# ScuffleCloud/SVT-AV1-mirror

Hardware: AMD Instinct MI355X
Metric: open-loop ME 64x64 superblocks/sec + achieved HBM GB/s, 4K preset-8 (higher is better)
Workload: dtype u8

## Files before the change

### include/svtme.h

```cpp
#ifndef SVTME_H
#define SVTME_H

#include <stdbool.h>
#include <stdint.h>

#ifdef __cplusplus
extern "C" {
#endif

#define SVTME_PU_COUNT 85
#define SVTME_MAX_LISTS 2
#define SVTME_MAX_REFS 4
#define SVTME_MAX_PA_ME_CAND 23
#define SVTME_MAX_PA_ME_MV 7
#define SVTME_MAX_SAD_VALUE (128u * 128u * 255u)
#define SVTME_SUB_SAD_SEARCH 0
#define SVTME_FULL_SAD_SEARCH 1
#define SVTME_ME_MCTF 1
#define SVTME_ME_OPEN_LOOP 3
#define SVTME_PAD_FULL 72
#define SVTME_PAD_QUARTER 32
#define SVTME_PAD_SIXTEENTH 16

typedef int32_t svtme_status;
// ... 202 lines not shown
svtme_status svtme_ticket_wait_timed(svtme_ctx *ctx, uint64_t ticket, float *gpu_ms, float *copy_ms);
void *svtme_host_alloc(uint64_t bytes);
void svtme_host_free(void *p);
svtme_status svtme_host_register(void *p, uint64_t bytes);
svtme_status svtme_host_unregister(void *p);
svtme_status svtme_reserve(svtme_ctx *ctx, uint32_t width, uint32_t height, uint32_t max_refs, uint32_t tickets);
svtme_status svtme_reserve_pictures(svtme_ctx *ctx, uint32_t width, uint32_t height, uint32_t count);
svtme_status svtme_set_timing(svtme_ctx *ctx, int enable);
uint32_t svtme_timing_read(svtme_ctx *ctx, float stage_ms[5]);
#define SVTME_PATH_NO_FUSED_HME 1u
#define SVTME_PATH_NO_L1_FULL 2u
#define SVTME_PATH_NO_L0_FULL 4u
#define SVTME_PATH_NO_FP_WIDE 8u
#define SVTME_PATH_SPLIT_PASS 16u
#define SVTME_PATH_NO_A1_GATE 32u
svtme_status svtme_set_paths(svtme_ctx *ctx, uint32_t paths);
void *svtme_device_records(svtme_ctx *ctx, uint64_t *bytes);
void *svtme_stream(svtme_ctx *ctx);

#define SVTME_DG_MAX_PAIRS 8
#define SVTME_DG_MAX_SA 128

typedef struct svtme_dg_pair {
    uint64_t cur_picture_number;
    uint64_t ref_picture_number;
} svtme_dg_pair;

typedef struct svtme_dg_sb {
    uint32_t sad;
    int16_t mv_x, mv_y;
// ... 118 lines not shown
```

### svt-av1-mirror_amd/csrc/svtme_host.cpp

```cpp
#include <hip/hip_runtime.h>

#include <algorithm>
#include <cstdarg>
#include <cstdio>
#include <cstdlib>
#include <chrono>
#include <condition_variable>
#include <cstring>
#include <map>
#include <mutex>
#include <string>
#include <vector>

#include "svtme_device.h"

extern "C" hipError_t svtme_launch_build_full(const void *src, uint32_t src_stride, int w, int h, int ten_bit,
                                              DevPlane dst, int left, int top, int rows, hipStream_t s);
extern "C" hipError_t svtme_launch_copy_words(const void *src, void *dst, uint32_t nwords, hipStream_t s);
extern "C" hipError_t svtme_launch_pack(const svtme_ref_record *d_recs, const svtme_sb_result *d_sb, uint32_t n_sb,
                                        uint32_t R, const svtme_pack_layout *L, void *d_out, hipStream_t s);
extern "C" hipError_t svtme_launch_build_down(DevPlane prev, DevPlane dst, int left, int top, int rows,
                                              hipStream_t s);
extern "C" hipError_t svtme_launch_stages(const DevJob *d_jobs, const DevJob *h_jobs, uint32_t n, hipStream_t s,
                                          hipEvent_t *ev, uint32_t *mask);
// ... 164 lines not shown
        return fail(SVTME_ERR_INSUFFICIENT_RESOURCES, "hipStreamCreate: %s", hipGetErrorString(e));
    }
    c->lanes[0].s = c->stream;
    if ((e = svtme_prime_pyramid()) != hipSuccess || (e = svtme_prime_pack()) != hipSuccess ||
        (e = svtme_prime_stages()) != hipSuccess || (e = svtme_prime_dg()) != hipSuccess ||
        (e = svtme_prime_tfsp()) != hipSuccess) {
        (void)hipStreamDestroy(c->stream);
        delete c;
        return fail(SVTME_ERR_UNDEFINED, "svtme_ctx_create: loading the kernels: %s", hipGetErrorString(e));
    }
    static const struct {
        const char *var;
        uint32_t bit;
    } env_paths[] = {{"SVTME_NO_FUSED_HME", SVTME_PATH_NO_FUSED_HME}, {"SVTME_NO_L1_FULL", SVTME_PATH_NO_L1_FULL},
                     {"SVTME_NO_L0_FULL", SVTME_PATH_NO_L0_FULL},       {"SVTME_NO_FP_WIDE", SVTME_PATH_NO_FP_WIDE},
                     {"SVTME_SPLIT_PASS", SVTME_PATH_SPLIT_PASS},     {"SVTME_NO_A1_GATE", SVTME_PATH_NO_A1_GATE}};
    for (const auto &e : env_paths)
        if (const char *v = getenv(e.var))
            if (*v && strcmp(v, "0") != 0)
                c->paths |= e.bit;
    if (const char *v = getenv("SVTME_UPLOAD_ZERO_COPY"))
        c->zero_copy = !(*v && strcmp(v, "0") == 0);
    const svtme_status ps = prepare(c);
    if (ps) {
        svtme_ctx_destroy(c);
        return ps;
    }
    *out = c;
    return SVTME_OK;
}

extern "C" svtme_status svtme_set_paths(svtme_ctx *c, uint32_t paths) {
    if (!c || (paths & ~63u))
        return fail(SVTME_ERR_BAD_PARAMETER, "svtme_set_paths: null ctx or unknown path bits 0x%x", paths);
    std::lock_guard<std::mutex> lk(c->mu);
    c->paths = paths;
    return SVTME_OK;
}

extern "C" void svtme_ctx_destroy(svtme_ctx *c) {
    if (!c)
        return;
    (void)hipSetDevice(c->device);
    for (auto &L : c->lanes)
        if (L.s)
            (void)hipStreamSynchronize(L.s);
    if (c->ustream)
        (void)hipStreamSynchronize(c->ustream);
// ... 1572 lines not shown
```

### svt-av1-mirror_amd/csrc/svtme_stages.hip

```cpp
#include <hip/hip_ext.h>
#include <cstdlib>
#include <type_traits>

#include "svtme_me_common.h"

extern "C" bool svtme_hme_rt(const svtme_controls *c);

namespace svtme {


#define STAGE_A_BUF_DW 1024
#define STAGE_B_BUF_DW 640

template <int ND, typename P>
__device__ __forceinline__ void rows_qsad(P rp, int bstride_dw, const uint8_t *src, int src_stride,
                                          int k0, int k1, uint32_t acc[4]) {
    constexpr int CH = 64 / ND;
    for (int kc = k0; kc < k1; kc += CH) {
        const int ke         = min(k1, kc + CH);
        unsigned long long a = 0;
#pragma unroll 2
        for (int k = kc; k < ke; k++) {
            const P rd         = rp + k * bstride_dw;
            const uint32_t *sd = (const uint32_t *)(src + k * src_stride);
// ... 1541 lines not shown
            const uint32_t cnt = (uint32_t)__builtin_popcount(cm);
            if (cnt < SVTME_MAX_PA_ME_CAND)
                ca[cnt] = 0;
            o->total_me_candidate_index[pu] = (uint8_t)cnt;
#pragma unroll
            for (int s2 = 0; s2 < 8; s2++) {
                if (!((slots >> s2) & 1u))
                    continue;
                uint32_t *dst = ((cm >> s2) & 1u) ? &o->me_mv_array[pu][(s2 >> 2 ? max_l0 : 0) + (s2 & 3)] : &st.sink;
                *dst          = mvs[s2];
            }
        }
    }
}

__device__ __forceinline__ void finish_sb_out(StC &st, const DevJob &dj, uint32_t sb_local, uint32_t bw, uint32_t bh) {
    static_assert(offsetof(svtme_sb_result, me_8x8_cost_variance) ==
                          offsetof(svtme_sb_result, me_distortion) + 4 * SVTME_PU_COUNT &&
                      offsetof(svtme_sb_result, stationary_block_present) ==
                          offsetof(svtme_sb_result, me_8x8_cost_variance) + 24 &&
                      sizeof(svtme_sb_result) == offsetof(svtme_sb_result, stationary_block_present) + 8,
                  "svtme_sb_result tail: 6 distortion words, then the GM flag bytes and padding");
    constexpr int NIMG = (int)(offsetof(svtme_sb_result, me_8x8_cost_variance) / 4);
    constexpr int WDIST = NIMG, WGM = NIMG + 6;
    const svtme_job &job = dj.job;
    const int tid = threadIdx.x, wid = tid >> 6, lane = tid & 63;
    const bool mctf = SF(job, me_type) == SVTME_ME_MCTF;
    const bool en8 = SF(job, enable_me_8x8) != 0, en16 = SF(job, enable_me_16x16) != 0;
    uint32_t *img      = (uint32_t *)&st.keys[0][0];
    svtme_sb_result *o = (svtme_sb_result *)img;
    uint32_t *ow       = (uint32_t *)(dj.out_sb + sb_local);
    if (wid >= 2) {
        const int t     = tid - 128;
        const int head  = (int)((16u - ((uint32_t)(uintptr_t)ow & 15u)) & 15u) >> 2;
        const int n16   = (NIMG - head) >> 2;
        const int tail0 = head + 4 * n16;
        for (int i = t; i < n16; i += 128) {
            const uint32_t *v = img + head + 4 * i;
            *(uint4 *)(ow + head + 4 * i) = make_uint4(v[0], v[1], v[2], v[3]);
        }
        if (t >= 128 - 8) {
            const int j = t - (128 - 8);
            if (j < head)
                ow[j] = img[j];
            else if (j >= 4 && tail0 + (j - 4) < NIMG)
                ow[tail0 + (j - 4)] = img[tail0 + (j - 4)];
        }
    } else if (wid == 0) {
        uint32_t w6 = 0;
        if (!mctf) {
            const uint32_t d8v  = o->me_distortion[21 + lane];
            const uint32_t d16v = lane < 16 ? o->me_distortion[5 + lane] : 0;
            const uint32_t d32v = lane < 4 ? o->me_distortion[1 + lane] : 0;
            const uint32_t d8 = wave_sum_u32(d8v), d16 = wave_sum_u32(d16v), d32 = wave_sum_u32(d32v);
            const uint32_t d64  = o->me_distortion[0];
            const uint64_t mean = d8 / 64;
            const int64_t diff  = (int64_t)d8v - (int64_t)mean;
            const uint64_t sq1  = (uint64_t)(diff * diff);
            const uint64_t sq   = ((uint64_t)wave_sum_u32((uint32_t)(sq1 >> 24)) << 24) +
                                (uint64_t)wave_sum_u32((uint32_t)(sq1 & 0xFFFFFFu));
            const uint32_t pix  = bw * bh;
            const uint32_t dd = lane == 2 ? d64 : lane == 3 ? d32 : lane == 4 ? d16 : d8;
// ... 53 lines not shown
                if (my < -active_th)
                    atomicAdd(&cnt[li][ri][1][0], 1u);
                else if (my > active_th)
                    atomicAdd(&cnt[li][ri][1][1], 1u);
                const int stt = low ? 0 : 4;
                stat          = absi(mx) <= stt && absi(my) <= stt;
            }
            const uint64_t stationary = (uint64_t)__popcll(__ballot(stat)), tot = (uint64_t)n_blk;
            wave_lds_fence();
            const bool over = lane < 32 && cntf[lane] > (tot / 2);
            const bool any  = __ballot(over) != 0ull;
            flags = (stationary > ((tot * 5) / 100) ? 1u : 0u) | (any ? 1u << 8 : 0u);
        }
        if (lane < 2)
            ow[WGM + lane] = lane == 0 ? flags : 0u;
    }}

__device__ __forceinline__ void finish_sb(StC &st, const DevJob &dj, uint32_t sb_local, uint32_t bw, uint32_t bh) {
    finish_sb_cands(st, dj, sb_local, bw, bh);
    __syncthreads();
    HME_SUB(20);
    finish_sb_out(st, dj, sb_local, bw, bh);
}

__device__ __forceinline__ void write_records(const StC &st, const DevJob &dj, uint32_t sb_local, int t, int nt) {
    static_assert(sizeof(svtme_ref_record) == 176 * 4, "svtme_ref_record: 176 dwords");
    svtme_ref_record *out = dj.out_records + (size_t)sb_local * dj.R;
    const int R = (int)dj.R, nr0 = (int)SF(dj.job, num_refs[0]);
    for (int i = t; i < R * 44; i += nt) {
        const int k = i / 44, q = i - 44 * k;
        const int s = k < nr0 ? k : 4 + (k - nr0);
        uint4 v     = ((const uint4 *)st.rec[s])[q];
        if (q < 22 && !st.searched[s]) {
            if (4 * q + 0 < 85) v.x = U32MAX;
            if (4 * q + 1 < 85) v.y = U32MAX;
            if (4 * q + 2 < 85) v.z = U32MAX;
            if (4 * q + 3 < 85) v.w = U32MAX;
        }
        if (q == 42) {
            v.z = (uint32_t)st.hme_sad[s];
            v.w = (uint32_t)(st.hme_sad[s] >> 32);
        } else if (q == 43) {
            v.x = (uint32_t)(uint16_t)st.sc_x[s] | ((uint32_t)(uint16_t)st.sc_y[s] << 16);
            v.y = st.zz[s];
            v.z = (uint32_t)st.searched[s] | ((uint32_t)st.do_ref[s] << 8) | ((uint32_t)st.tf_exit << 16);
            v.w = 0;
        }
        ((uint4 *)(out + k))[q] = v;
    }
}

template <bool SUMS>
__device__ __forceinline__ void stage_c_tail(StC &st, const DevJob &dj, uint32_t sb_local, uint32_t bw, uint32_t bh, uint32_t vmask) {
    const svtme_job &job    = dj.job;
    const svtme_controls &c = job.ctrl;
    const int tid = threadIdx.x, lane = tid & 63;
    const bool w0 = (tid >> 6) == 0;
    const bool sbr = dj.out_sb != nullptr;
    uint32_t *img  = (uint32_t *)&st.keys[0][0];
    if (SF(job, me_type) != SVTME_ME_MCTF && SF(c, enable_hme_flag) && SF(c, enable_me_hme_ref_pruning) && w0) {
        const int s = lane;
        uint32_t sum8 = 0;
        if (SUMS) {
            if (s < 8)
                sum8 = st.sum8[s];
        } else {
            for (int k = 0; k < 8; k++) {
                if (!(slot_valid(vmask, k) && st.do_ref[k]))
                    continue;
                const uint32_t t = wave_sum_u32(st.rec[k][21 + lane]);
// ... 5 lines not shown
        if (s < 8) {
            v = st.hme_sad[s];
            if (slot_valid(vmask, s)) {
                v             = st.do_ref[s] ? (uint64_t)sum8 : (uint64_t)SVTME_MAX_SAD_VALUE * 64;
                st.hme_sad[s] = v;
            }
        }
        const uint16_t th = (uint16_t)SF(c, prune_ref_if_me_sad_dev_bigger_than_th);
        if (th != (uint16_t)~0) {
            const uint64_t best = wave_min_u64(v);
            if (s < 8 && (s & 3) >= 1 && (v - best) * 100 > (th * best))
                st.do_ref[s] = 0;
        }
    }
    if (SUMS && sbr && !w0)
        for (int i = tid - 64; i < (int)(sizeof(svtme_sb_result) + 15) / 16; i += 192)
            ((uint4 *)img)[i] = make_uint4(0, 0, 0, 0);
    __syncthreads();
    HME_SUB(17);
    if (SUMS && sbr) {
        if (tid < 128)
            finish_sb_cands(st, dj, sb_local, bw, bh);
        else
            write_records(st, dj, sb_local, tid - 128, 128);
        HME_SUB(18);
        __syncthreads();
        HME_SUB(20);
        finish_sb_out(st, dj, sb_local, bw, bh);
        HME_SUB(21);
        return;
    }
    write_records(st, dj, sb_local, tid, 256);
    HME_SUB(18);
    if (sbr) {
        for (int i = tid; i < (int)(sizeof(svtme_sb_result) + 15) / 16; i += 256)
            ((uint4 *)img)[i] = make_uint4(0, 0, 0, 0);
        __syncthreads();
        HME_SUB(19);
        finish_sb(st, dj, sb_local, bw, bh);
        HME_SUB(21);
    }
}

template <bool SUB_ME>
__global__ void __launch_bounds__(256) __attribute__((amdgpu_waves_per_eu(4, 8))) k_stage_c(const DevBatch B) {
    __shared__ StC st;
    uint32_t sb_local;
    const DevJob &dj        = batch_job(B, xcd_remap(blockIdx.x, gridDim.x), &sb_local);
    const svtme_job &job    = dj.job;
    const svtme_controls &c = job.ctrl;
    const int tid = threadIdx.x, lane = tid & 63, wid = tid >> 6;
    const bool w0           = wid == 0;
    const SbGeo G           = sb_geo(dj, sb_local);
    const uint32_t ox = G.ox, oy = G.oy, bw = G.bw, bh = G.bh;
// ... 650 lines not shown
    put(k8, 21 + lane);
    if ((lane & 3) == 0)
        put(k16, 5 + (lane >> 2));
    if ((lane & 15) == 0)
        put(k32, 1 + (lane >> 4));
    if (lane == 63)
        put(k64, 0);
    if (lane < 6) {
        const uint32_t t[6] = {(uint32_t)v.hme_sad, (uint32_t)(v.hme_sad >> 32),
                               (uint32_t)(uint16_t)v.sc_x | ((uint32_t)(uint16_t)v.sc_y << 16), v.zz,
                               (uint32_t)v.searched | ((uint32_t)v.do_ref << 8) | ((uint32_t)v.tf_exit << 16), 0u};
        o[170 + lane] = t[lane];
    }
}

template <bool SUB, bool K32, int TQ = (SUB ? FP_TQ : 2), bool WIDE = false, int WHOLE = 7>
__device__ __forceinline__ void fp_slot(const DevJob &dj, const SbGeo &G, int s, const uint32_t (&src)[SUB ? 4 : 8][2],
                                        int by, int bx, uint64_t hme_sad, uint32_t zz, uint32_t rdiv, int16_t sc_x,
                                        int16_t sc_y, uint8_t dref, uint8_t tf_exit, int part, uint32_t parts,
                                        unsigned long long *kp, CSlot *cs, svtme_ref_record *rec = nullptr) {
    const int lane = threadIdx.x & 63;
    const int l = s >> 2, r = s & 3;
    const uint32_t ox = G.ox, oy = G.oy;
    if (!dref || tf_exit) {
        const CSlot cv{hme_sad, zz, sc_x, sc_y, 0, 0, 0, 0, 0, 0, dref, 0, tf_exit};
        if (part == 0 && lane == 0)
            *cs = cv;
        if (rec)
            direct_record(rec, cv, 0, 0, 0, 0);
        return;
    }
    const DevPlane &P = dj.ref[l][r].lv[0];
    PuMin<K32> M;
    M.clear();
    const FpArea A = fp_area(dj, G, s, zz, rdiv, sc_x, sc_y, [&](const uint8_t *g) {
        const int sh = (int)((uintptr_t)g & 3);
        uint32_t p8, p64;
        if constexpr (K32) {
            p8  = fp_probe32<SUB>(M, g, P.stride >> 2, src, by, bx);
            p64 = wave_sum_u32(p8);
// ... 838 lines not shown
    if (search) {
        uint32_t bs;
        int x, y;
        key_result(half ? kt : kb, &bs, &x, &y);
        SD = bs;
        X  = i16((x + xo) * 2);
        Y  = i16((y + yo) * 2);
    }
    if ((lane & 47) == 0) {
        b->hx[s][q]   = X;
        b->hy[s][q]   = Y;
        b->hsad[s][q] = SD;
    }
}

__device__ __forceinline__ void stage_e_body(StC &st, const DevJob &dj, uint32_t sb_local,
                                             const SbGeo &G, uint32_t vmask, const CSlot *cin,
                                             unsigned long long *kb, bool reset) {
    const svtme_job &job = dj.job;
    const int tid = threadIdx.x, wid = tid >> 6, lane = tid & 63;
    const int R = (int)dj.R, nr0 = (int)SF(job, num_refs[0]);
    if (tid < 8) {
        const int s    = tid;
        const int k    = s < 4 ? s : nr0 + (s - 4);
        const bool has = s < 4 ? s < nr0 : k < R;
        CSlot v{};
        if (has)
            v = cin[k];
        st.hme_sad[s]  = has ? v.hme_sad : U32MAX;
        st.zz[s]       = has ? v.zz : U32MAX;
        st.sc_x[s]     = has ? v.sc_x : 0;
        st.sc_y[s]     = has ? v.sc_y : 0;
        st.searched[s] = has ? v.searched : 0;
        st.do_ref[s]   = has ? v.do_ref : 0;
        if (!(has && v.searched))
            st.sum8[s] = 0;
        if (s == (nr0 > 0 ? 0 : 4))
            st.tf_exit = has ? v.tf_exit : 0;
    }
    for (int kk = wid; kk < R; kk += 4) {
        const int s      = kk < nr0 ? kk : 4 + (kk - nr0);
        const CSlot &v   = cin[kk];
        const bool srch  = v.searched != 0;
        const uint32_t wm = srch ? magic_u32((uint32_t)max(1, (int)v.w)) : 0u;
        auto decode = [&](int pu, uint32_t &sad, uint32_t &mv) {
            sad = U32MAX, mv = 0;
            if (srch) {
                const size_t e                = (size_t)kk * SVTME_PU_COUNT + pu;
                const unsigned long long key = kb[e];
                if (reset)
                    kb[e] = ~0ull;
                const uint32_t o = (uint32_t)key;
                sad              = (uint32_t)(key >> 32);
                int16_t mx, my;
                if (v.probe && o == 0) {
// ... 9 lines not shown
            }
            st.rec[s][pu]                  = sad;
            st.rec[s][SVTME_PU_COUNT + pu] = mv;
        };
        uint32_t sad, mv;
        decode(21 + lane, sad, mv);
        if (srch) {
            const uint32_t t = wave_sum_u32(sad);
            if (lane == 0)
                st.sum8[s] = t;
        }
        if (lane < 21)
            decode(lane, sad, mv);
    }
    __syncthreads();
    stage_c_tail<true>(st, dj, sb_local, G.bw, G.bh, vmask);
}

__global__ void __launch_bounds__(256) __attribute__((amdgpu_waves_per_eu(4, 8))) k_stage_e(const DevBatch B) {
    __shared__ StC st;
    uint32_t sb_local;
    const DevJob &dj     = batch_job(B, xcd_remap(blockIdx.x, gridDim.x), &sb_local);
    const SbGeo G        = sb_geo(dj, sb_local);
    const uint32_t vmask = valid_mask(dj.job);
    stage_e_body(st, dj, sb_local, G, vmask, dj.cslot + (size_t)sb_local * dj.R,
                 dj.keys + (size_t)sb_local * dj.R * SVTME_PU_COUNT, dj.parts > 1);
}

struct HmeA {
    Dec d;
    unsigned long long key[SVTME_A_N];
// ... 126 lines not shown
struct HmeSh {
    DevJob dj;
    BState bs;
    CSlot cin[8];
    SlotCentre cen[8];
    uint8_t tf_exit;
    union U {
        HmeA a;
        StC st;
    } u;
};

#define HME_PRIO_HI() __builtin_amdgcn_s_setprio(2)
#define HME_PRIO_LO() __builtin_amdgcn_s_setprio(0)
#define HME_WAVES_PER_EU 8
template <bool FP, bool SUB_ME, bool K32, bool RT = false>
__global__ void __launch_bounds__(256) __attribute__((amdgpu_waves_per_eu(HME_WAVES_PER_EU, HME_WAVES_PER_EU))) k_hme(const DevBatch B) {
    __shared__ HmeSh sh;
    const int tid = threadIdx.x, lane = tid & 63, wid = UNI(tid >> 6);
    uint32_t sb_local;
    const DevJob &gj = batch_job(B, xcd_remap(blockIdx.x, gridDim.x), &sb_local);
    {
        static_assert(sizeof(DevJob) % 16 == 0 && sizeof(DevJob) / 16 <= 256, "DevJob: one uint4 per thread");
        if (tid < (int)(sizeof(DevJob) / 16))
            ((uint4 *)&sh.dj)[tid] = ((const uint4 *)&gj)[tid];
    }
    __syncthreads();
    const DevJob &dj        = sh.dj;
    const svtme_job &job    = dj.job;
    const svtme_controls &c = job.ctrl;
    const SbGeo G           = sb_geo(dj, sb_local);
    const uint32_t vmask    = valid_mask(job);
    Dec &d                  = sh.u.a.d;
    const int16_t sox = i16(((int16_t)G.ox) >> 2), soy = i16(((int16_t)G.oy) >> 2);
    const int kh  = (int)(G.bh >> 2) >> 1;
    const int kh1 = (int)(G.bh >> 2);
    const bool zz_on = c.me_early_exit_th || c.me_safe_limit_zz_th;
    HME_STAMP(0);

    if (wid == 0) {
// ... 86 lines not shown
        const bool act    = lane < 16 && slot_valid(vmask, s) && tl_or_l0(job, s >> 2) && ds;
        const bool nd     = act && ((lane & 1) ? !(eet && zs < (eet >> 2)) : !(eet && zs < eet));
        const unsigned long long m = __ballot(nd);
        if (lane == 0)
            sh.u.a.need = (uint32_t)m;
        HME_PRIO_LO();
    } else if (wid == 1) {
        if (lane < SVTME_A_N)
            sh.u.a.key[lane] = ~0ull;
        const bool gate = !RT && c.prehme_enable && c.prehme_l1_early_exit && job.num_lists == 2 &&
                          c.hme_search_method != SVTME_FULL_SAD_SEARCH && !(dj.paths & SVTME_PATH_NO_A1_GATE);
        a1_table<RT ? 1 : 0>(sh.u.a, dj, vmask, sox, soy, kh, 0, 0, 0, gate);
    } else {
        if (c.enable_hme_level2_flag) {
            const DevPlane &F = dj.cur.lv[0];
            const int row = (tid - 128) >> 2, part = tid & 3;
            const u32x4a4 v = ldg4((const uint32_t *)(F.base + (ptrdiff_t)(G.oy + 2 * row) * F.stride + G.ox + 16 * part));
            ((uint4 *)sh.u.a.src1[row])[part] = make_uint4(v.x, v.y, v.z, v.w);
        }
        if (c.enable_hme_level1_flag && tid < 160) {
            const DevPlane &Q = dj.cur.lv[1];
            const int row = (tid - 128) >> 1, half = tid & 1;
            const u32x4a4 v = ldg4((const uint32_t *)(Q.base + (ptrdiff_t)((G.oy >> 1) + 2 * row) * Q.stride +
                                                      (G.ox >> 1) + 16 * half));
            ((uint4 *)sh.u.a.src4[row])[half] = make_uint4(v.x, v.y, v.z, v.w);
        }
    }
    HME_WAVE(0);
    __syncthreads();
    HME_STAMP(1);
    HME_STAMP(2);
    auto a1_tiles = [&]() {
        uint32_t sr[8][4];
        {
            const uint8_t *sp = uni_ptr(dj.cur.lv[2].base + (ptrdiff_t)soy * dj.cur.lv[2].stride + sox);
            const int sst     = UNI(dj.cur.lv[2].stride);
#pragma unroll
            for (int k = 0; k < 8; k++) {
                const uint4 v = sld4(sp + (ptrdiff_t)(2 * k) * sst);
                sr[k][0] = v.x, sr[k][1] = v.y, sr[k][2] = v.z, sr[k][3] = v.w;
            }
        }
        const int nitems = sh.u.a.nitems, nsrch = sh.u.a.nsrch;
        const uint32_t need = sh.u.a.need;
        const int pstride = dj.cur.lv[2].stride;
        const int nitems3 = sh.u.a.nitems3, base2 = sh.u.a.base2, end1 = sh.u.a.end1, base3 = sh.u.a.base3;
        auto tiles = [&](auto fullk, int lo, int hi, bool gated) {
            for (int it = lo + tid; it < hi; it += 256) {
                if (it >= nitems3 && it < base2)
                    continue;
                const HSrch &e = sh.u.a.srch[find_search(sh.u.a.srch, nsrch, it)];
                if (!((need >> e.need) & 1u))
                    continue;
                if (gated && a1_mirrored(sh.u.a, c, need, e.id))
                    continue;
                const int local = it - e.item0;
                const int rt = mdiv(local, e.ncm), col = local - rt * e.ncols;
                auto run = [&](auto TT) {
                    constexpr int T = decltype(TT)::value;
                    int yf, tv;
                    if (e.skip) {
                        yf = 2 * T * rt + 1;
                        tv = min(T, e.cnt0 - T * rt);
// ... 236 lines not shown
            e.item0     = incl - items;
            sh.u.a.s1[kpos] = e;
        }
        if (lane == 63)
            sh.u.a.nitems1 = incl;
        if (lane == 0)
            sh.u.a.nsrch1 = tot;
    }
    __syncthreads();
    HME_PRIO_LO();
    HME_STAMP(4);
    {
        const int nlanes = 4 * sh.u.a.nitems1, nsrch = sh.u.a.nsrch1;
        const int pstride = dj.cur.lv[1].stride;
        auto tiles = [&](auto fullk) {
            for (int it4 = tid; it4 < nlanes; it4 += 256) {
                const int it    = it4 >> 2;
                const HSrch1 &e = sh.u.a.s1[find_search(sh.u.a.s1, nsrch, it)];
                const int local = it - e.item0;
                const int y = mdiv(local, e.ncm), col = local - y * e.ncols;
                const unsigned long long kk = hme_tile32q<decltype(fullk)::value>(e.a0, pstride, HQ1 * col, e.sh,
                                                                                  e.sa_w, y, kh1, sh.u.a.src4);
                if ((it4 & 3) == 0 && kk != ~0ull)
                    atomicMin(&sh.u.a.key1[e.id], kk);
            }
        };
        tiles(std::false_type());
    }
    __syncthreads();
    if (wid == 0 && lane < 32 && sh.u.a.hsad[lane] == ~0ull) {
        uint32_t best;
// ... 40 lines not shown
            const int incl = wave_incl_scan(items);
            if (mk) {
                e.item0            = incl - items;
                sh.u.a.s1[kpos] = e;
            }
            if (lane == 63)
                sh.u.a.nitems1 = incl;
            if (lane == 0)
                sh.u.a.nsrch1 = tot;
        }
        __syncthreads();
        {
            const int nlanes = 8 * sh.u.a.nitems1, nsrch = sh.u.a.nsrch1;
            const int pstride = dj.cur.lv[0].stride;
            const int kh2     = (int)(G.bh >> 1);
            for (int it8 = tid; it8 < nlanes; it8 += 256) {
                const int it    = it8 >> 3;
                const HSrch1 &e = sh.u.a.s1[find_search(sh.u.a.s1, nsrch, it)];
                const int local = it - e.item0;
                const int y = mdiv(local, e.ncm), col = local - y * e.ncols;
                const unsigned long long kk = hme_tile64(e.a0, pstride, HQ * col, e.sh, e.sa_w, y, kh2, sh.u.a.src1);
                if ((it8 & 7) == 0 && kk != ~0ull)
                    atomicMin(&sh.u.a.key1[e.id], kk);
            }
        }
        __syncthreads();
        if (wid == 0 && lane < 32 && sh.u.a.hsad[lane] == ~0ull) {
            uint32_t best;
            int x, y;
            key_result(sh.u.a.key1[lane], &best, &x, &y);
            sh.u.a.hsad[lane] = hsub ? (uint64_t)best * 2 : best;
// ... 21 lines not shown
        HME_STAMP(6);
        return;
    }
    if (wid == 0) {
        HME_PRIO_HI();
        wave_lds_fence();
        const SlotCentre scv = final_centre(gj.job, &sh.bs, vmask);
        if (lane < 8)
            sh.cen[lane] = scv;
        if (lane == 0)
            sh.tf_exit = job.me_type == SVTME_ME_MCTF && scv.hme_sad < job.tf_me_exit_th;
    }
    __syncthreads();
    HME_PRIO_LO();
    HME_STOP(55);
    for (int k = wid; k < (int)dj.R; k += 4) {
        constexpr int ROWS = SUB_ME ? 4 : 8, RSTEP = SUB_ME ? 2 : 1;
        int fl = lane;
        asm volatile("" : "+v"(fl));
        const int z16 = fl >> 2, k4 = fl & 3;
        const int by  = ((z16 >> 3) << 2) | (((z16 >> 1) & 1) << 1) | (k4 >> 1);
        const int bx  = (((z16 >> 2) & 1) << 2) | ((z16 & 1) << 1) | (k4 & 1);
        const DevPlane &C = gj.cur.lv[0];
        const int cst     = UNI(C.stride);
        const __amdgpu_buffer_rsrc_t crs = plane_rsrc(uni_ptr(C.base + (ptrdiff_t)G.oy * cst + G.ox));
        const uint32_t coff = (uint32_t)(by * 8 * cst + bx * 8);
        uint32_t src[ROWS][2];
#pragma unroll
        for (int rr = 0; rr < ROWS; rr++) {
            const auto v = __builtin_amdgcn_raw_buffer_load_b64(crs, (int)coff, rr * RSTEP * cst, 0);
            src[rr][0] = v[0];
            src[rr][1] = v[1];
        }
        const int nr0       = (int)SF(gj.job, num_refs[0]);
        const int s         = k < nr0 ? k : 4 + (k - nr0);
        const SlotCentre &v = sh.cen[s];
        fp_slot<SUB_ME, K32, 2, false, HME_WHOLE>(gj, G, s, src, by, bx, rl64(v.hme_sad, 0), (uint32_t)UNI(v.zz), (uint32_t)UNI(v.reduce_div),
                                (int16_t)UNI(v.sc_x), (int16_t)UNI(v.sc_y), (uint8_t)UNI(v.do_ref),
                                (uint8_t)UNI(sh.tf_exit), 0, 1u, &sh.u.st.keys[k][0], &sh.cin[k]);
    }
    HME_WAVE(1);
    __syncthreads();
    HME_STAMP(6);
    stage_e_body(sh.u.st, gj, sb_local, G, vmask, sh.cin, &sh.u.st.keys[0][0], false);
    HME_STAMP(7);
}

}

extern "C" void svtme_stage_a_list(const svtme_job *job, uint8_t *list, uint32_t *count) {
    const svtme_controls &c = job->ctrl;
    uint32_t n = 0;
    for (int s = 0; s < 8; s++) {
        const int l = s >> 2, r = s & 3;
        if (l >= job->num_lists || r >= job->num_refs[l])
            continue;
        if (!(job->temporal_layer_index > 0 || l == 0))
            continue;
        const bool zz = c.me_early_exit_th || c.me_safe_limit_zz_th;
// ... 72 lines not shown
        for (int k = 0; k < 2; k++) {
            const uint32_t mw = (uint32_t)c.prehme_sa_cfg[k].sa_min.width * f, xw = c.prehme_sa_cfg[k].sa_max.width;
            const uint32_t mh = (uint32_t)c.prehme_sa_cfg[k].sa_min.height * f, xh = c.prehme_sa_cfg[k].sa_max.height;
            dj->ph_sa[s][k][0] = (int16_t)(uint16_t)(mw < xw ? mw : xw);
            dj->ph_sa[s][k][1] = (int16_t)(uint16_t)(mh < xh ? mh : xh);
        }
    }
}

extern "C" bool svtme_hme_fused(const svtme_job *job) {
    const svtme_controls &c = job->ctrl;
    return (job->width % 64) == 0 && c.hme_search_method != SVTME_FULL_SAD_SEARCH;
}
static bool hme_fused(const DevJob &dj) { return svtme_hme_fused(&dj.job) && !(dj.paths & SVTME_PATH_NO_FUSED_HME); }

extern "C" bool svtme_hme_rt(const svtme_controls *c) {
    return c->enable_me_sr_adjustment && c->distance_based_hme_resizing && c->reduce_hme_l0_sr_th_min &&
           c->reduce_hme_l0_sr_th_max;
}

extern "C" bool svtme_l1_full(const svtme_controls *c) {
    return c->hme_search_method == SVTME_FULL_SAD_SEARCH && c->enable_hme_flag && c->enable_hme_level1_flag &&
           !c->enable_hme_level2_flag && c->hme_l1_sa.width <= 16 && c->hme_l1_sa.height <= 16;
}
static bool l1_full(const DevJob &dj) { return svtme_l1_full(&dj.job.ctrl) && !(dj.paths & SVTME_PATH_NO_L1_FULL); }

extern "C" bool svtme_l0_full(const DevJob *dj) {
    const svtme_controls &c = dj->job.ctrl;
    if (c.hme_search_method != SVTME_FULL_SAD_SEARCH || c.prehme_enable || !c.enable_hme_flag ||
        !c.enable_hme_level0_flag || svtme_hme_rt(&c) || (dj->job.width % 64) % 16 != 0 ||
// ... 53 lines not shown
    if (fp_wide_lds(c, paths)) {
        parts = parts > (h + 7) / 8 ? parts : (h + 7) / 8;
        parts = (parts + 3) & ~3u;
    }
    return parts < 1 ? 1 : (parts > 16 ? 16 : parts);
}
extern "C" uint32_t svtme_fp_parts(const svtme_controls *c) { return svtme_fp_parts_paths(c, 0); }

extern "C" uint32_t svtme_launch_key(const DevJob *dj) {
    const bool full = dj->job.ctrl.me_search_method == SVTME_FULL_SAD_SEARCH;
    return (uint32_t)full | (uint32_t)(dj->parts != 0) << 1 | (uint32_t)svtme_fp_k32(&dj->job.ctrl) << 2 |
           (uint32_t)(dj->job.ctrl.enable_hme_level2_flag != 0) << 3 | (uint32_t)hme_fused(*dj) << 4 |
           (uint32_t)(dj->parts == 1) << 5 | (uint32_t)svtme_fp_wide(&dj->job.ctrl) << 6 |
           (uint32_t)svtme_hme_rt(&dj->job.ctrl) << 7 | (uint32_t)fp_wide_lds(*dj) << 8 |
           (uint32_t)l1_full(*dj) << 9 | (uint32_t)svtme_l0_full(dj) << 10 |
           (uint32_t)((dj->paths & SVTME_PATH_SPLIT_PASS) != 0) << 11;
}

static DevBatch make_batch(const DevJob *d_jobs, const DevJob *h, uint32_t n, uint32_t (*units)(const DevJob &)) {
    DevBatch b;
    b.jobs     = d_jobs;
    b.n        = n;
    uint32_t t = 0;
    for (uint32_t k = 0; k < SVTME_MAX_BATCH; k++) {
        b.start[k] = k < n ? t : 0xFFFFFFFFu;
        if (k < n)
            t += units(h[k]);
    }
    b.total = t;
    return b;
}

#define SVTME_LAUNCH(K, grid, k, ...)                                                                               \
    do {                                                                                                           \
        if (ev) {                                                                                                  \
            hipExtLaunchKernelGGL(K, grid, dim3(256), 0, s, ev[2 * (k)], ev[2 * (k) + 1], 0, __VA_ARGS__);           \
            *mask |= 1u << (k);                                                                                    \
        } else                                                                                                     \
            hipLaunchKernelGGL(K, grid, dim3(256), 0, s, __VA_ARGS__);                                             \
    } while (0)

extern "C" hipError_t svtme_prime_stages(void) {
    const void *k[] = {
        (const void *)svtme::k_hme<true, true, true, false>,   (const void *)svtme::k_hme<true, true, true, true>,
        (const void *)svtme::k_hme<false, true, true, false>,  (const void *)svtme::k_hme<true, true, false, false>,
        (const void *)svtme::k_stage_a<false>,                 (const void *)svtme::k_stage_a<true>,
        (const void *)svtme::k_stage_d<false>,                 (const void *)svtme::k_stage_d<true>,
        (const void *)svtme::k_stage_b<false>,                 (const void *)svtme::k_stage_b<true>,
        (const void *)svtme::k_stage_c<false>,                 (const void *)svtme::k_stage_c<true>,
        (const void *)svtme::k_stage_c1<true, true, true>,     (const void *)svtme::k_stage_c1<true, true>,
        (const void *)svtme::k_stage_c1<true, false>,          (const void *)svtme::k_stage_c1<false, true, true>,
        (const void *)svtme::k_stage_c1<false, true>,          (const void *)svtme::k_stage_c1<false, false>,
        (const void *)svtme::k_l0_full<2>,                     (const void *)svtme::k_l0_full<4>,
        (const void *)svtme::k_l1_full,                        (const void *)svtme::k_fp_wide,
        (const void *)svtme::k_stage_e};
    hipFuncAttributes a;
    for (const void *f : k) {
        const hipError_t e = hipFuncGetAttributes(&a, f);
        if (e != hipSuccess)
            return e;
// ... 8 lines not shown
    const DevJob &h0 = h_jobs[0];
    if (mask)
        *mask = 0;
    const DevBatch bd = make_batch(d_jobs, h_jobs, n, [](const DevJob &j) { return j.job.sb_count; });
    const bool full = h0.job.ctrl.me_search_method == SVTME_FULL_SAD_SEARCH;
    const bool k32  = svtme_fp_k32(&h0.job.ctrl);
    const bool rt = svtme_hme_rt(&h0.job.ctrl);
#define SVTME_HME(FP, SUB, K32)                                                                                     \
    do {                                                                                                           \
        if (rt)                                                                                                    \
            SVTME_LAUNCH((svtme::k_hme<FP, SUB, K32, true>), dim3(bd.total), 0, bd);                               \
        else                                                                                                       \
            SVTME_LAUNCH((svtme::k_hme<FP, SUB, K32, false>), dim3(bd.total), 0, bd);                              \
    } while (0)
    if (hme_fused(h0) && h0.parts == 1 && !(h0.paths & SVTME_PATH_SPLIT_PASS)) {
        if (full && k32)
            SVTME_HME(true, false, true);
        else if (full)
            SVTME_HME(true, false, false);
        else if (k32)
            SVTME_HME(true, true, true);
        else
            SVTME_HME(true, true, false);
        return hipGetLastError();
    }
    if (hme_fused(h0)) {
        SVTME_HME(false, true, true);
    } else {
    const DevBatch ba = make_batch(d_jobs, h_jobs, n, [](const DevJob &j) { return j.job.sb_count * j.ta_count; });
    bool short_l0 = true;
    for (uint32_t k = 0; k < n; k++)
// ... 63 lines not shown
```

### svt-av1-mirror_amd/svtme.py

```python
from __future__ import annotations

import ctypes as C
import os
from dataclasses import dataclass, field

import numpy as np

PKG_DIR = os.path.dirname(os.path.abspath(__file__))
REPO_DIR = os.path.dirname(PKG_DIR)

PU_COUNT = 85
MAX_SAD_VALUE = 128 * 128 * 255
MAX_TICKETS = 64
PAD_FULL, PAD_QUARTER, PAD_SIXTEENTH = 72, 32, 16
SUB_SAD_SEARCH, FULL_SAD_SEARCH = 0, 1
ME_MCTF, ME_OPEN_LOOP = 1, 3
PATH_NO_FUSED_HME, PATH_NO_L1_FULL, PATH_NO_L0_FULL, PATH_NO_FP_WIDE, PATH_SPLIT_PASS = 1, 2, 4, 8, 16
RES_240P, RES_360P, RES_480P, RES_720P, RES_1080P, RES_4K, RES_8K = range(7)


class Area(C.Structure):
    _fields_ = [("width", C.c_uint16), ("height", C.c_uint16)]


class AreaMinMax(C.Structure):
    _fields_ = [("sa_min", Area), ("sa_max", Area)]


class Controls(C.Structure):
    _fields_ = [
        ("hme_search_method", C.c_uint8),
        ("me_search_method", C.c_uint8),
# ... 893 lines not shown
```

Before: 68.62 million.

## Launch fused HME kernel with three wavefronts for sub-SAD low-ref jobs

Adds a 3-wavefront (192-thread) variant of the fused HME kernel, used by default for sub-SAD, non-RT jobs with at most four references. Work loops, the image store, record writes and the source loads are made generic over the wave count. Full-pel slot assignment now hands searched references round-robin to waves and gives unsearched slots to the last wave, so idle waves are not spent on them. The aim is more resident workgroups per CU with less idle-wave waste, at the cost of fewer threads per block for the per-SB tail work and a new HME_4WAVES opt-out flag.

```diff
diff --git a/include/svtme.h b/include/svtme.h
--- a/include/svtme.h
+++ b/include/svtme.h
@@ -240,6 +240,7 @@
 #define SVTME_PATH_NO_FP_WIDE 8u
 #define SVTME_PATH_SPLIT_PASS 16u
 #define SVTME_PATH_NO_A1_GATE 32u
+#define SVTME_PATH_HME_4WAVES 64u
 svtme_status svtme_set_paths(svtme_ctx *ctx, uint32_t paths);
 void *svtme_device_records(svtme_ctx *ctx, uint64_t *bytes);
 void *svtme_stream(svtme_ctx *ctx);
diff --git a/svt-av1-mirror_amd/csrc/svtme_host.cpp b/svt-av1-mirror_amd/csrc/svtme_host.cpp
--- a/svt-av1-mirror_amd/csrc/svtme_host.cpp
+++ b/svt-av1-mirror_amd/csrc/svtme_host.cpp
@@ -202,7 +202,8 @@
         uint32_t bit;
     } env_paths[] = {{"SVTME_NO_FUSED_HME", SVTME_PATH_NO_FUSED_HME}, {"SVTME_NO_L1_FULL", SVTME_PATH_NO_L1_FULL},
                      {"SVTME_NO_L0_FULL", SVTME_PATH_NO_L0_FULL},       {"SVTME_NO_FP_WIDE", SVTME_PATH_NO_FP_WIDE},
-                     {"SVTME_SPLIT_PASS", SVTME_PATH_SPLIT_PASS},     {"SVTME_NO_A1_GATE", SVTME_PATH_NO_A1_GATE}};
+                     {"SVTME_SPLIT_PASS", SVTME_PATH_SPLIT_PASS},     {"SVTME_NO_A1_GATE", SVTME_PATH_NO_A1_GATE},
+                     {"SVTME_HME_4WAVES", SVTME_PATH_HME_4WAVES}};
     for (const auto &e : env_paths)
         if (const char *v = getenv(e.var))
             if (*v && strcmp(v, "0") != 0)
@@ -219,7 +220,7 @@
 }
 
 extern "C" svtme_status svtme_set_paths(svtme_ctx *c, uint32_t paths) {
-    if (!c || (paths & ~63u))
+    if (!c || (paths & ~127u))
         return fail(SVTME_ERR_BAD_PARAMETER, "svtme_set_paths: null ctx or unknown path bits 0x%x", paths);
     std::lock_guard<std::mutex> lk(c->mu);
     c->paths = paths;
diff --git a/svt-av1-mirror_amd/csrc/svtme_stages.hip b/svt-av1-mirror_amd/csrc/svtme_stages.hip
--- a/svt-av1-mirror_amd/csrc/svtme_stages.hip
+++ b/svt-av1-mirror_amd/csrc/svtme_stages.hip
@@ -1579,6 +1579,7 @@
     }
 }
 
+template <int NW = 4>
 __device__ __forceinline__ void finish_sb_out(StC &st, const DevJob &dj, uint32_t sb_local, uint32_t bw, uint32_t bh) {
     static_assert(offsetof(svtme_sb_result, me_8x8_cost_variance) ==
                           offsetof(svtme_sb_result, me_distortion) + 4 * SVTME_PU_COUNT &&
@@ -1595,8 +1596,7 @@
     uint32_t *img      = (uint32_t *)&st.keys[0][0];
     svtme_sb_result *o = (svtme_sb_result *)img;
     uint32_t *ow       = (uint32_t *)(dj.out_sb + sb_local);
-    if (wid >= 2) {
-        const int t     = tid - 128;
+    auto store_image = [&](int t) {
         const int head  = (int)((16u - ((uint32_t)(uintptr_t)ow & 15u)) & 15u) >> 2;
         const int n16   = (NIMG - head) >> 2;
         const int tail0 = head + 4 * n16;
@@ -1611,6 +1611,9 @@
             else if (j >= 4 && tail0 + (j - 4) < NIMG)
                 ow[tail0 + (j - 4)] = img[tail0 + (j - 4)];
         }
+    };
+    if (wid >= 2) {
+        store_image(tid - 128);
     } else if (wid == 0) {
         uint32_t w6 = 0;
         if (!mctf) {
@@ -1694,13 +1697,17 @@
         }
         if (lane < 2)
             ow[WGM + lane] = lane == 0 ? flags : 0u;
-    }}
-
+        if (NW == 3)
+            store_image(64 + lane);
+    }
+}
+
+template <int NW = 4>
 __device__ __forceinline__ void finish_sb(StC &st, const DevJob &dj, uint32_t sb_local, uint32_t bw, uint32_t bh) {
     finish_sb_cands(st, dj, sb_local, bw, bh);
     __syncthreads();
     HME_SUB(20);
-    finish_sb_out(st, dj, sb_local, bw, bh);
+    finish_sb_out<NW>(st, dj, sb_local, bw, bh);
 }
 
 __device__ __forceinline__ void write_records(const StC &st, const DevJob &dj, uint32_t sb_local, int t, int nt) {
@@ -1730,10 +1737,11 @@
     }
 }
 
-template <bool SUMS>
+template <bool SUMS, int NW = 4>
 __device__ __forceinline__ void stage_c_tail(StC &st, const DevJob &dj, uint32_t sb_local, uint32_t bw, uint32_t bh, uint32_t vmask) {
     const svtme_job &job    = dj.job;
     const svtme_controls &c = job.ctrl;
+    constexpr int NT = 64 * NW;
     const int tid = threadIdx.x, lane = tid & 63;
     const bool w0 = (tid >> 6) == 0;
     const bool sbr = dj.out_sb != nullptr;
@@ -1769,7 +1777,7 @@
         }
     }
     if (SUMS && sbr && !w0)
-        for (int i = tid - 64; i < (int)(sizeof(svtme_sb_result) + 15) / 16; i += 192)
+        for (int i = tid - 64; i < (int)(sizeof(svtme_sb_result) + 15) / 16; i += NT - 64)
             ((uint4 *)img)[i] = make_uint4(0, 0, 0, 0);
     __syncthreads();
     HME_SUB(17);
@@ -1777,22 +1785,22 @@
         if (tid < 128)
             finish_sb_cands(st, dj, sb_local, bw, bh);
         else
-            write_records(st, dj, sb_local, tid - 128, 128);
+            write_records(st, dj, sb_local, tid - 128, NT - 128);
         HME_SUB(18);
         __syncthreads();
         HME_SUB(20);
-        finish_sb_out(st, dj, sb_local, bw, bh);
+        finish_sb_out<NW>(st, dj, sb_local, bw, bh);
         HME_SUB(21);
         return;
     }
-    write_records(st, dj, sb_local, tid, 256);
+    write_records(st, dj, sb_local, tid, NT);
     HME_SUB(18);
     if (sbr) {
-        for (int i = tid; i < (int)(sizeof(svtme_sb_result) + 15) / 16; i += 256)
+        for (int i = tid; i < (int)(sizeof(svtme_sb_result) + 15) / 16; i += NT)
             ((uint4 *)img)[i] = make_uint4(0, 0, 0, 0);
         __syncthreads();
         HME_SUB(19);
-        finish_sb(st, dj, sb_local, bw, bh);
+        finish_sb<NW>(st, dj, sb_local, bw, bh);
         HME_SUB(21);
     }
 }
@@ -2473,6 +2481,11 @@
     }
 }
 
+__device__ __forceinline__ CSlot fp_unsearched(uint64_t hme_sad, uint32_t zz, int16_t sc_x, int16_t sc_y, uint8_t dref,
+                                               uint8_t tf_exit) {
+    return CSlot{hme_sad, zz, sc_x, sc_y, 0, 0, 0, 0, 0, 0, dref, 0, tf_exit};
+}
+
 template <bool SUB, bool K32, int TQ = (SUB ? FP_TQ : 2), bool WIDE = false, int WHOLE = 7>
 __device__ __forceinline__ void fp_slot(const DevJob &dj, const SbGeo &G, int s, const uint32_t (&src)[SUB ? 4 : 8][2],
                                         int by, int bx, uint64_t hme_sad, uint32_t zz, uint32_t rdiv, int16_t sc_x,
@@ -2482,7 +2495,7 @@
     const int l = s >> 2, r = s & 3;
     const uint32_t ox = G.ox, oy = G.oy;
     if (!dref || tf_exit) {
-        const CSlot cv{hme_sad, zz, sc_x, sc_y, 0, 0, 0, 0, 0, 0, dref, 0, tf_exit};
+        const CSlot cv = fp_unsearched(hme_sad, zz, sc_x, sc_y, dref, tf_exit);
         if (part == 0 && lane == 0)
             *cs = cv;
         if (rec)
@@ -3351,6 +3364,7 @@
     }
 }
 
+template <int NW = 4>
 __device__ __forceinline__ void stage_e_body(StC &st, const DevJob &dj, uint32_t sb_local,
                                              const SbGeo &G, uint32_t vmask, const CSlot *cin,
                                              unsigned long long *kb, bool reset) {
@@ -3375,7 +3389,7 @@
         if (s == (nr0 > 0 ? 0 : 4))
             st.tf_exit = has ? v.tf_exit : 0;
     }
-    for (int kk = wid; kk < R; kk += 4) {
+    for (int kk = wid; kk < R; kk += NW) {
         const int s      = kk < nr0 ? kk : 4 + (kk - nr0);
         const CSlot &v   = cin[kk];
         const bool srch  = v.searched != 0;
@@ -3415,7 +3429,7 @@
             decode(lane, sad, mv);
     }
     __syncthreads();
-    stage_c_tail<true>(st, dj, sb_local, G.bw, G.bh, vmask);
+    stage_c_tail<true, NW>(st, dj, sb_local, G.bw, G.bh, vmask);
 }
 
 __global__ void __launch_bounds__(256) __attribute__((amdgpu_waves_per_eu(4, 8))) k_stage_e(const DevBatch B) {
@@ -3572,16 +3586,21 @@
 #define HME_PRIO_HI() __builtin_amdgcn_s_setprio(2)
 #define HME_PRIO_LO() __builtin_amdgcn_s_setprio(0)
 #define HME_WAVES_PER_EU 8
-template <bool FP, bool SUB_ME, bool K32, bool RT = false>
-__global__ void __launch_bounds__(256) __attribute__((amdgpu_waves_per_eu(HME_WAVES_PER_EU, HME_WAVES_PER_EU))) k_hme(const DevBatch B) {
+template <bool FP, bool SUB_ME, bool K32, bool RT = false, int NW = 4>
+__global__ void __launch_bounds__(64 * NW) __attribute__((amdgpu_waves_per_eu(HME_WAVES_PER_EU, HME_WAVES_PER_EU))) k_hme(const DevBatch B) {
+    static_assert(NW == 3 || NW == 4, "k_hme: 3 or 4 wavefronts");
+    static_assert(sizeof(HmeSh) <= 16384, "HmeSh: ten workgroups per CU (160 KB of LDS)");
+    constexpr int NT = 64 * NW;
     __shared__ HmeSh sh;
     const int tid = threadIdx.x, lane = tid & 63, wid = UNI(tid >> 6);
     uint32_t sb_local;
     const DevJob &gj = batch_job(B, xcd_remap(blockIdx.x, gridDim.x), &sb_local);
     {
-        static_assert(sizeof(DevJob) % 16 == 0 && sizeof(DevJob) / 16 <= 256, "DevJob: one uint4 per thread");
+        static_assert(sizeof(DevJob) % 16 == 0 && sizeof(DevJob) / 16 <= 2 * NT, "DevJob: at most two uint4 per thread");
         if (tid < (int)(sizeof(DevJob) / 16))
             ((uint4 *)&sh.dj)[tid] = ((const uint4 *)&gj)[tid];
+        if (sizeof(DevJob) / 16 > NT && tid + NT < (int)(sizeof(DevJob) / 16))
+            ((uint4 *)&sh.dj)[tid + NT] = ((const uint4 *)&gj)[tid + NT];
     }
     __syncthreads();
     const DevJob &dj        = sh.dj;
@@ -3698,9 +3717,18 @@
     } else {
         if (c.enable_hme_level2_flag) {
             const DevPlane &F = dj.cur.lv[0];
-            const int row = (tid - 128) >> 2, part = tid & 3;
-            const u32x4a4 v = ldg4((const uint32_t *)(F.base + (ptrdiff_t)(G.oy + 2 * row) * F.stride + G.ox + 16 * part));
-            ((uint4 *)sh.u.a.src1[row])[part] = make_uint4(v.x, v.y, v.z, v.w);
+            constexpr int NP = 128 / (NT - 128);
+            u32x4a4 v[NP];
+#pragma unroll
+            for (int p = 0; p < NP; p++) {
+                const int i = tid - 128 + p * (NT - 128), row = i >> 2, part = i & 3;
+                v[p] = ldg4((const uint32_t *)(F.base + (ptrdiff_t)(G.oy + 2 * row) * F.stride + G.ox + 16 * part));
+            }
+#pragma unroll
+            for (int p = 0; p < NP; p++) {
+                const int i = tid - 128 + p * (NT - 128), row = i >> 2, part = i & 3;
+                ((uint4 *)sh.u.a.src1[row])[part] = make_uint4(v[p].x, v[p].y, v[p].z, v[p].w);
+            }
         }
         if (c.enable_hme_level1_flag && tid < 160) {
             const DevPlane &Q = dj.cur.lv[1];
@@ -3730,7 +3758,7 @@
         const int pstride = dj.cur.lv[2].stride;
         const int nitems3 = sh.u.a.nitems3, base2 = sh.u.a.base2, end1 = sh.u.a.end1, base3 = sh.u.a.base3;
         auto tiles = [&](auto fullk, int lo, int hi, bool gated) {
-            for (int it = lo + tid; it < hi; it += 256) {
+            for (int it = lo + tid; it < hi; it += NT) {
                 if (it >= nitems3 && it < base2)
                     continue;
                 const HSrch &e = sh.u.a.srch[find_search(sh.u.a.srch, nsrch, it)];
@@ -3997,7 +4025,7 @@
         const int nlanes = 4 * sh.u.a.nitems1, nsrch = sh.u.a.nsrch1;
         const int pstride = dj.cur.lv[1].stride;
         auto tiles = [&](auto fullk) {
-            for (int it4 = tid; it4 < nlanes; it4 += 256) {
+            for (int it4 = tid; it4 < nlanes; it4 += NT) {
                 const int it    = it4 >> 2;
                 const HSrch1 &e = sh.u.a.s1[find_search(sh.u.a.s1, nsrch, it)];
                 const int local = it - e.item0;
@@ -4068,7 +4096,7 @@
             const int nlanes = 8 * sh.u.a.nitems1, nsrch = sh.u.a.nsrch1;
             const int pstride = dj.cur.lv[0].stride;
             const int kh2     = (int)(G.bh >> 1);
-            for (int it8 = tid; it8 < nlanes; it8 += 256) {
+            for (int it8 = tid; it8 < nlanes; it8 += NT) {
                 const int it    = it8 >> 3;
                 const HSrch1 &e = sh.u.a.s1[find_search(sh.u.a.s1, nsrch, it)];
                 const int local = it - e.item0;
@@ -4120,8 +4148,22 @@
     __syncthreads();
     HME_PRIO_LO();
     HME_STOP(55);
-    for (int k = wid; k < (int)dj.R; k += 4) {
+    const int nrec = (int)dj.R, nr0 = (int)SF(gj.job, num_refs[0]);
+    const uint8_t tfx = (uint8_t)UNI(sh.tf_exit);
+    for (int k = 0, j = 0; k < nrec; k++) {
         constexpr int ROWS = SUB_ME ? 4 : 8, RSTEP = SUB_ME ? 2 : 1;
+        const int s         = k < nr0 ? k : 4 + (k - nr0);
+        const SlotCentre &v = sh.cen[s];
+        const bool srch     = UNI(v.do_ref) && !tfx;
+        const int owner     = srch ? j : NW - 1;
+        j                   = srch ? (j + 1 == NW ? 0 : j + 1) : j;
+        if (wid != owner)
+            continue;
+        if (!srch) {
+            if (lane == 0)
+                sh.cin[k] = fp_unsearched(v.hme_sad, v.zz, v.sc_x, v.sc_y, v.do_ref, tfx);
+            continue;
+        }
         int fl = lane;
         asm volatile("" : "+v"(fl));
         const int z16 = fl >> 2, k4 = fl & 3;
@@ -4138,17 +4180,14 @@
             src[rr][0] = v[0];
             src[rr][1] = v[1];
         }
-        const int nr0       = (int)SF(gj.job, num_refs[0]);
-        const int s         = k < nr0 ? k : 4 + (k - nr0);
-        const SlotCentre &v = sh.cen[s];
         fp_slot<SUB_ME, K32, 2, false, HME_WHOLE>(gj, G, s, src, by, bx, rl64(v.hme_sad, 0), (uint32_t)UNI(v.zz), (uint32_t)UNI(v.reduce_div),
-                                (int16_t)UNI(v.sc_x), (int16_t)UNI(v.sc_y), (uint8_t)UNI(v.do_ref),
-                                (uint8_t)UNI(sh.tf_exit), 0, 1u, &sh.u.st.keys[k][0], &sh.cin[k]);
+                                (int16_t)UNI(v.sc_x), (int16_t)UNI(v.sc_y), (uint8_t)UNI(v.do_ref), tfx, 0, 1u,
+                                &sh.u.st.keys[k][0], &sh.cin[k]);
     }
     HME_WAVE(1);
     __syncthreads();
     HME_STAMP(6);
-    stage_e_body(sh.u.st, gj, sb_local, G, vmask, sh.cin, &sh.u.st.keys[0][0], false);
+    stage_e_body<NW>(sh.u.st, gj, sb_local, G, vmask, sh.cin, &sh.u.st.keys[0][0], false);
     HME_STAMP(7);
 }
 
@@ -4251,6 +4290,21 @@
 }
 static bool hme_fused(const DevJob &dj) { return svtme_hme_fused(&dj.job) && !(dj.paths & SVTME_PATH_NO_FUSED_HME); }
 
+extern "C" uint32_t svtme_hme_waves(const svtme_job *job) {
+    const svtme_controls &c = job->ctrl;
+    uint32_t R = 0;
+    for (int l = 0; l < job->num_lists && l < 2; l++) R += job->num_refs[l];
+    return c.me_search_method != SVTME_FULL_SAD_SEARCH && !svtme_hme_rt(&c) && R <= 4 ? 3u : 4u;
+}
+extern "C" uint32_t svtme_hme_waves_paths(const svtme_job *job, uint32_t paths) {
+    return (paths & SVTME_PATH_HME_4WAVES) ? 4u : svtme_hme_waves(job);
+}
+static uint32_t hme_waves(const DevJob &dj) {
+    const bool whole = svtme_hme_fused(&dj.job) && dj.parts == 1 &&
+                       !(dj.paths & (SVTME_PATH_NO_FUSED_HME | SVTME_PATH_SPLIT_PASS));
+    return whole ? svtme_hme_waves_paths(&dj.job, dj.paths) : 4u;
+}
+
 extern "C" bool svtme_hme_rt(const svtme_controls *c) {
     return c->enable_me_sr_adjustment && c->distance_based_hme_resizing && c->reduce_hme_l0_sr_th_min &&
            c->reduce_hme_l0_sr_th_max;
@@ -4334,7 +4388,7 @@
            (uint32_t)(dj->parts == 1) << 5 | (uint32_t)svtme_fp_wide(&dj->job.ctrl) << 6 |
            (uint32_t)svtme_hme_rt(&dj->job.ctrl) << 7 | (uint32_t)fp_wide_lds(*dj) << 8 |
            (uint32_t)l1_full(*dj) << 9 | (uint32_t)svtme_l0_full(dj) << 10 |
-           (uint32_t)((dj->paths & SVTME_PATH_SPLIT_PASS) != 0) << 11;
+           (uint32_t)((dj->paths & SVTME_PATH_SPLIT_PASS) != 0) << 11 | (uint32_t)(hme_waves(*dj) == 3) << 12;
 }
 
 static DevBatch make_batch(const DevJob *d_jobs, const DevJob *h, uint32_t n, uint32_t (*units)(const DevJob &)) {
@@ -4351,19 +4405,21 @@
     return b;
 }
 
-#define SVTME_LAUNCH(K, grid, k, ...)                                                                               \
+#define SVTME_LAUNCH_NT(K, grid, nt, k, ...)                                                                        \
     do {                                                                                                           \
         if (ev) {                                                                                                  \
-            hipExtLaunchKernelGGL(K, grid, dim3(256), 0, s, ev[2 * (k)], ev[2 * (k) + 1], 0, __VA_ARGS__);           \
+            hipExtLaunchKernelGGL(K, grid, dim3(nt), 0, s, ev[2 * (k)], ev[2 * (k) + 1], 0, __VA_ARGS__);            \
             *mask |= 1u << (k);                                                                                    \
         } else                                                                                                     \
-            hipLaunchKernelGGL(K, grid, dim3(256), 0, s, __VA_ARGS__);                                             \
+            hipLaunchKernelGGL(K, grid, dim3(nt), 0, s, __VA_ARGS__);                                              \
     } while (0)
+#define SVTME_LAUNCH(K, grid, k, ...) SVTME_LAUNCH_NT(K, grid, 256, k, __VA_ARGS__)
 
 extern "C" hipError_t svtme_prime_stages(void) {
     const void *k[] = {
         (const void *)svtme::k_hme<true, true, true, false>,   (const void *)svtme::k_hme<true, true, true, true>,
         (const void *)svtme::k_hme<false, true, true, false>,  (const void *)svtme::k_hme<true, true, false, false>,
+        (const void *)svtme::k_hme<true, true, true, false, 3>, (const void *)svtme::k_hme<true, true, false, false, 3>,
         (const void *)svtme::k_stage_a<false>,                 (const void *)svtme::k_stage_a<true>,
         (const void *)svtme::k_stage_d<false>,                 (const void *)svtme::k_stage_d<true>,
         (const void *)svtme::k_stage_b<false>,                 (const void *)svtme::k_stage_b<true>,
@@ -4402,7 +4458,11 @@
             SVTME_LAUNCH((svtme::k_hme<FP, SUB, K32, false>), dim3(bd.total), 0, bd);                              \
     } while (0)
     if (hme_fused(h0) && h0.parts == 1 && !(h0.paths & SVTME_PATH_SPLIT_PASS)) {
-        if (full && k32)
+        if (hme_waves(h0) == 3 && k32)
+            SVTME_LAUNCH_NT((svtme::k_hme<true, true, true, false, 3>), dim3(bd.total), 192, 0, bd);
+        else if (hme_waves(h0) == 3)
+            SVTME_LAUNCH_NT((svtme::k_hme<true, true, false, false, 3>), dim3(bd.total), 192, 0, bd);
+        else if (full && k32)
             SVTME_HME(true, false, true);
         else if (full)
             SVTME_HME(true, false, false);
diff --git a/svt-av1-mirror_amd/svtme.py b/svt-av1-mirror_amd/svtme.py
--- a/svt-av1-mirror_amd/svtme.py
+++ b/svt-av1-mirror_amd/svtme.py
@@ -16,6 +16,7 @@
 SUB_SAD_SEARCH, FULL_SAD_SEARCH = 0, 1
 ME_MCTF, ME_OPEN_LOOP = 1, 3
 PATH_NO_FUSED_HME, PATH_NO_L1_FULL, PATH_NO_L0_FULL, PATH_NO_FP_WIDE, PATH_SPLIT_PASS = 1, 2, 4, 8, 16
+PATH_NO_A1_GATE, PATH_HME_4WAVES = 32, 64
 RES_240P, RES_360P, RES_480P, RES_720P, RES_1080P, RES_4K, RES_8K = range(7)
 
 
```

New measurement: 72.97 million (median of 6 runs). 6.3% higher.
